# ctu-mrs/mrs_uav_trajectory_generation

Hardware: NVIDIA B200
Metric: optimized+sampled trajectories/sec (10-seg, N=10, fp64) (higher is better)
Workload: dtype f64

## Files before the change

### mrs_uav_trajectory_generation_b200/csrc/cuda_backend.cu

```cuda
#include <cuda_runtime.h>

#include <cub/device/device_scan.cuh>
#include <cub/device/device_select.cuh>
#include <cub/iterator/counting_input_iterator.cuh>
#include <chrono>
#include <cstdlib>
#include <cstring>
#include <map>
#include <mutex>
#include <utility>
#include <vector>
#include <stdexcept>
#include <string>
#include <typeinfo>

#define TG_VERSION_STRING "tg_b200 0.1.0 (sm_100a, fp64, -fmad=false)"

#ifndef TG_JT_REFILL_REP
#define TG_JT_REFILL_REP 2
#endif
#include "tg_kernels.cuh"

namespace {

// ... 2 lines not shown
    cudaError_t e__ = (expr);                                                                            \
    if (e__ != cudaSuccess)                                                                              \
      throw std::runtime_error(std::string(#expr) + ": " + cudaGetErrorString(e__));                     \
  } while (0)

template <class F, class = void>
struct MinBlocksOf {
  static constexpr int value = 1;
};
template <class F>
struct MinBlocksOf<F, decltype((void)F::kMinBlocks)> {
  static constexpr int value = F::kMinBlocks;
};
template <class F>
__global__ void __launch_bounds__(128, MinBlocksOf<F>::value) k_for_each(const F f, const size_t n) {
  const size_t i = (size_t)blockIdx.x * blockDim.x + threadIdx.x;
  if (i < n) f(i);
}

template <class F>
__global__ void __launch_bounds__(128) k_for_each_warp(const F f, const size_t n) {
  const size_t w = (size_t)blockIdx.x * 4 + (threadIdx.x >> 5);
  if (w < n) f(w, (int)(threadIdx.x & 31));
}

static_assert(TG_WARR_DEVICE_STRIDE == 32, "strided scratch kernels run one warp per block");
template <class F>
__global__ void __launch_bounds__(TG_WARR_DEVICE_STRIDE) k_for_each_scratch(const F f, const size_t n) {
  extern __shared__ double smem[];
  const size_t i = (size_t)blockIdx.x * blockDim.x + threadIdx.x;
  if (i < n) f(i, smem + threadIdx.x, (int)blockDim.x);
}

constexpr int kSolveWarps = 4;
template <class D>
__global__ void __launch_bounds__(kSolveWarps * 32) k_solve(const D desc, const size_t inst_begin, const size_t n_inst, const int ws_doubles, double* __restrict__ gws,
                                                            const int skip_oct_ws, const bool skip_thread) {
  extern __shared__ double smem[];
  const int warp = threadIdx.x >> 5, lane = threadIdx.x & 31;
  const size_t gw = (size_t)blockIdx.x * kSolveWarps + warp, nw = (size_t)gridDim.x * kSolveWarps;
  double* ws = gws ? gws + gw * (size_t)ws_doubles : smem + (size_t)warp * ws_doubles;
  for (size_t inst = inst_begin + gw; inst < n_inst; inst += nw) {
    tg::SolveInst I;
    if (!desc.instance(inst, I)) continue;
    if (skip_thread && tg::thread_eligible(I)) continue;
    if (skip_oct_ws > 0 && tg::octet_eligible(I) && tg::octet_ws_doubles(I.S, I.np) <= skip_oct_ws) continue;
// ... 411 lines not shown
    return (double)ms;
  }

  template <class F>
  void for_each(size_t n, const F& f) {
    if (n == 0) return;
    const unsigned block = 128;
    const size_t grid = (n + block - 1) / block;
    prof_begin();
    k_for_each<F><<<(unsigned)grid, block, 0, stream>>>(f, n);
    TG_CUDA_CHECK(cudaGetLastError());
    prof_end(typeid(F).name(), n);
  }
  template <class F>
  void for_each_warp(size_t n, const F& f) {
    if (n == 0) return;
    const size_t grid = (n + 3) / 4;
    prof_begin();
    k_for_each_warp<F><<<(unsigned)grid, 128, 0, stream>>>(f, n);
    TG_CUDA_CHECK(cudaGetLastError());
    prof_end(typeid(F).name(), n);
  }
  template <class F>
  void for_each_scratch(size_t n, const F& f) {
    if (n == 0) return;
    const unsigned block = TG_WARR_DEVICE_STRIDE;
    const size_t grid = (n + block - 1) / block;
    const size_t smem = (size_t)F::kScratch * sizeof(double) * block;
    allow_smem((const void*)k_for_each_scratch<F>, smem);
    prof_begin();
    k_for_each_scratch<F><<<(unsigned)grid, block, smem, stream>>>(f, n);
    TG_CUDA_CHECK(cudaGetLastError());
    prof_end(typeid(F).name(), n);
  }
  void fork(int n) {
    if (profiling) return;
    TG_CUDA_CHECK(cudaEventRecord(ev_fork, stream));
    for (int i = 0; i < n && i < kSideStreams; ++i) TG_CUDA_CHECK(cudaStreamWaitEvent(side[i], ev_fork, 0));
  }
  void join(int n) {
    if (profiling) return;
    for (int i = 0; i < n && i < kSideStreams; ++i) {
      TG_CUDA_CHECK(cudaEventRecord(ev_side[i], side[i]));
      TG_CUDA_CHECK(cudaStreamWaitEvent(stream, ev_side[i], 0));
    }
  }
// ... 293 lines not shown
```

### mrs_uav_trajectory_generation_b200/csrc/tg_kernels.cuh

```cuda
#ifndef TG_KERNELS_CUH_
#define TG_KERNELS_CUH_

#include "tg_common.cuh"
#include "tg_bound.cuh"
#include "tg_plis.cuh"
#include "tg_node.cuh"
#include "tg_poly.cuh"
#include "tg_segment.cuh"
#include "tg_solve.cuh"
#include "tg_solve_octet.cuh"
#include "tg_solve_thread.cuh"

#if defined(__CUDA_ARCH__)
#define TG_ATOMIC_MAX(p, v) atomicMax((p), (v))
#define TG_ATOMIC_ADD(p, v) atomicAdd((p), (v))
#define TG_ATOMIC_ADD_RET(p, v) atomicAdd((p), (v))
#elif defined(__CUDACC__)
#define TG_ATOMIC_MAX(p, v) ((void)0)
#define TG_ATOMIC_ADD(p, v) ((void)0)
#define TG_ATOMIC_ADD_RET(p, v) (0)
#else
static inline void tg_host_atomic_max(int* p, int v) {
  int cur = __atomic_load_n(p, __ATOMIC_RELAXED);
  while (cur < v && !__atomic_compare_exchange_n(p, &cur, v, true, __ATOMIC_RELAXED, __ATOMIC_RELAXED)) {
// ... 25 lines not shown
  double max_dev;
};

struct BatchPtrs {
  int B, totS, totV, r;
  const int* seg_off;
  const int* prob_of_vtx;
  const int* prob_of_seg;
  const double* wp;
  const uint8_t* stop;
  const double* init14;
  uint8_t* vmask;
  double* vval;
  int* vfree;
  int* np;
  int* hbw;
  int* fmax;
  int* stats;
  double *times, *baca, *xeval, *x, *g, *d, *hist_s, *hist_y;
  PlisScalars* opt;
  int* ix;
  int* act_prob[2];
  int* act_vtx[2];
  int* act_seg[2];
  double* recs;
  double* costs;
  double* coef;
  double* maxima;
  ProbState* ps;
  double* xs;
  double* part;
  int xstride, smax;
};

TG_HD int vtx_off(const BatchPtrs& b, int p) { return b.seg_off[p] + p; }

struct PrepareFn {
  BatchPtrs b;
  int from_waypoints;
  TG_HD void operator()(size_t pi) const {
    const int p = (int)pi, s0 = b.seg_off[p], S = b.seg_off[p + 1] - s0, V = S + 1, v0 = s0 + p;
    int hbw = 0, np;
    if (from_waypoints)
      np = build_vertices(V, b.wp + 4 * (size_t)v0, b.stop ? b.stop + v0 : nullptr, b.init14 ? b.init14 + 14 * (size_t)p : nullptr, b.r,
                          b.vmask + v0, b.vval + (size_t)v0 * TG_HALF * TG_D, b.vfree + v0 + p, &hbw);
    else
      np = index_vertices(V, b.vmask + v0, b.vfree + v0 + p, &hbw);
// ... 36 lines not shown
    const int p = b.prob_of_seg[gs];
    const int s0 = b.seg_off[p], S = b.seg_off[p + 1] - s0, i = (int)gs - s0, v0 = s0 + p;
    const double* vpos = b.vval + (size_t)v0 * TG_HALF * TG_D;
    const int stride = TG_HALF * TG_D;
    b.times[gs] = segment_time_euclidean(vpos + (size_t)i * stride, vpos + (size_t)(i + 1) * stride, L);
    b.baca[gs] = segment_time_baca(vpos, stride, i, S + 1, L);
  }
};
struct BacaTotalFn {
  BatchPtrs b;
  TG_HD void operator()(size_t pi) const {
    const int p = (int)pi, s0 = b.seg_off[p], S = b.seg_off[p + 1] - s0;
    double tot = 0.0;
    for (int i = 0; i < S; ++i) tot = tot + b.baca[s0 + i];
    b.ps[p].baca_total = tot;
  }
};

struct SetupBaseFn {
  BatchPtrs b;
  const double* T;
  TG_HD void operator()(size_t gs) const { setup_segment_record(T[gs], b.r, b.recs + gs * TG_REC_SIZE); }
};
template <int STAGE>
struct SetupMellingerFn {
  BatchPtrs b;
  const int* seg_list;
  static constexpr int stage = STAGE;
#ifndef TG_SETUP_ROW_BLOCKS
#define TG_SETUP_ROW_BLOCKS 8
#endif
  static constexpr int kMinBlocks = STAGE ? TG_SETUP_ROW_BLOCKS : 2;
  TG_HD void operator()(size_t item00) const {
    const size_t item0 = stage ? item00 / TG_N : item00;
    const size_t k = item0 / 3;
    const int which = (int)(item0 - k * 3);
    const size_t gs = seg_list ? (size_t)seg_list[k] : k;
    const size_t item = gs * 3 + which;
    const int p = b.prob_of_seg[gs];
    double T = stage ? 0.0 : b.xeval[gs];
    if (b.opt[p].done) return;
    const int S = b.seg_off[p + 1] - b.seg_off[p];
    if (S == 1 && which != 0) return;
    double* rec = b.recs + item * TG_REC_SIZE;
    if (stage) {
      setup_record_hrow(b.r, rec, (int)(item00 - item0 * TG_N));
      return;
    }
    if (which == 1) {
      T = T + 0.1;
      T = dmax(kTimeLowerBound, T);
    } else if (which == 2) {
      const double corr = 0.1 / ((double)S - 1.0);
      T = T - corr;
      T = dmax(kTimeLowerBound, T);
    }
    setup_record_head(T, b.r, rec);
  }
};

struct SolveProblemDesc {
  BatchPtrs b;
  int mellinger;
  double* dp_out;
  const int* dp_off;
  TG_HD bool instance(size_t inst, SolveInst& I) const {
    int p, n;
    if (mellinger == 1) {
      p = b.prob_of_vtx[inst];
      n = (int)inst - vtx_off(b, p);
      if (b.opt[p].done) return false;
    } else {
      p = (int)inst;
      n = 0;
    }
    const int s0 = b.seg_off[p], S = b.seg_off[p + 1] - s0, v0 = s0 + p;
    if (mellinger && S == 1 && n > 0) return false;
    I.S = S;
    I.np = b.np[p];
    I.hbw = b.hbw[p];
// ... 174 lines not shown
    SolveInst I;
    if (!desc.instance(inst, I)) return;
    if (it >= I.S * TG_D) return;
    run_instance(I, inst * (size_t)per_inst + it, it);
  }
  TG_HD void run_instance(const SolveInst& I, size_t item, int it) const {
    const int s = it >> 2, d = it & 3;
    const double* rec = solve_rec(I, s);
    double nd[TG_N], c[TG_N];
#pragma unroll
    for (int k = 0; k < TG_N; ++k) {
      const int v = s + (k >= TG_HALF ? 1 : 0), sl = k - (k >= TG_HALF ? TG_HALF : 0);
      const uint32_t m = I.vmask[v];
      nd[k] = ((m >> sl) & 1u) ? I.vval[((size_t)v * TG_HALF + sl) * TG_D + d] : I.x_out[(size_t)(I.vfree[v] + free_rank(m, sl)) * 4 + d];
    }
    coef_from_endpoints(rec, nd, c);
    if (I.coef_out) {
#pragma unroll
      for (int a = 0; a < TG_N; a += 2) store2(I.coef_out + it * TG_N + a, c[a], c[a + 1]);
    }
    if (I.cost_out) part[item] = cost_partial_rec(I.r, c, rec);
  }
};
struct CoefCostGradFn {
#ifndef TG_COEF_MIN_BLOCKS
#define TG_COEF_MIN_BLOCKS 5
#endif
  static constexpr int kMinBlocks = TG_COEF_MIN_BLOCKS;
  CoefCostFn<SolveProblemDesc> f;
  int p0;
  const int* prob_list;
  TG_HD void operator()(size_t item0) const {
    const BatchPtrs& b = f.desc.b;
    const int p = prob_list ? prob_list[item0 >> 7] : p0 + (int)(item0 >> 7), t = (int)(item0 & 127);
    if (b.opt[p].done) return;
    const int s0 = b.seg_off[p], S = b.seg_off[p + 1] - s0, v0 = s0 + p;
    const int per = S * TG_D, total = (S == 1) ? per : (S + 1) * per;
    SolveInst I;
    I.S = S;
    I.np = 0;
    I.hbw = 0;
    I.fmax = 0;
    I.rec_stride = 3;
    I.r = b.r;
    I.vmask = b.vmask + v0;
    I.vfree = b.vfree + v0 + p;
    I.vval = b.vval + (size_t)v0 * TG_HALF * TG_D;
    I.recs = b.recs + (size_t)s0 * 3 * TG_REC_SIZE;
    I.dp_out = nullptr;
    for (int k = t; k < total; k += 128) {
      const int n = k / per, it = k - n * per;
      I.variant = n;
      I.coef_out = (n == 0) ? b.coef + (size_t)s0 * TG_D * TG_N : nullptr;
      I.cost_out = b.costs + v0 + n;
      I.x_out = b.xs + (size_t)(v0 + n) * (size_t)b.xstride;
      f.run_instance(I, (size_t)(v0 + n) * (size_t)f.per_inst + it, it);
    }
  }
};
template <class D>
struct CostSumFn {
  D desc;
  int per_inst;
  const double* part;
  const int* inst_list = nullptr;
  TG_HD void operator()(size_t k) const {
    const size_t inst = inst_list ? (size_t)inst_list[k] : k;
    SolveInst I;
    if (!desc.instance(inst, I)) return;
    if (!I.cost_out) return;
    const double* pp = part + inst * (size_t)per_inst;
    double total = 0.0;
    for (int it = 0; it < I.S * TG_D; ++it) total += pp[it];
    *I.cost_out = 0.5 * total;
  }
};

TG_HD PlisVectors plis_vectors(const BatchPtrs& b, int p) {
  PlisVectors v;
  const int s0 = b.seg_off[p];
  v.x = b.x + s0;
  v.gf = b.g + s0;
  v.s = b.d + s0;
  v.xeval = b.xeval + s0;
  v.xo = b.hist_s + s0;
  v.go = b.hist_y + s0;
  v.ix = b.ix + s0;
  v.hstride = (size_t)b.totS;
  return v;
}
TG_HD void plis_enlist(const BatchPtrs& b, int p, int buf) {
  const int s0 = b.seg_off[p], S = b.seg_off[p + 1] - s0, v0 = s0 + p;
  int* cnt = b.stats + 9 + 3 * buf;
  const int jp = TG_ATOMIC_ADD_RET(&cnt[0], 1);
  b.act_prob[buf][jp] = p;
  const int jv = TG_ATOMIC_ADD_RET(&cnt[1], S + 1);
  for (int n = 0; n <= S; ++n) b.act_vtx[buf][jv + n] = v0 + n;
  const int js = TG_ATOMIC_ADD_RET(&cnt[2], S);
  for (int i = 0; i < S; ++i) b.act_seg[buf][js + i] = s0 + i;
}
struct PlisBeginFn {
  BatchPtrs b;
  int max_evals;
  TG_HD void operator()(size_t pi) const {
    const int p = (int)pi, s0 = b.seg_off[p], S = b.seg_off[p + 1] - s0;
    if (plis_begin(S, b.opt[p], plis_vectors(b, p), b.times + s0, max_evals)) plis_enlist(b, p, 0);
  }
};
struct PlisAdvanceFn {
  BatchPtrs b;
  int max_evals;
  double f_rel, x_rel;
  const int* prob_list;
  int next_buf;
  TG_HD void operator()(size_t k) const {
    const int p = prob_list ? prob_list[k] : (int)k, s0 = b.seg_off[p], S = b.seg_off[p + 1] - s0;
    PlisScalars& st = b.opt[p];
    if (st.done) return;
    plis_advance(S, st, plis_vectors(b, p), b.costs + vtx_off(b, p), max_evals, f_rel, x_rel, -1.0);
    if (!st.done) {
      TG_ATOMIC_ADD(&b.stats[7], 1);
      plis_enlist(b, p, next_buf);
    }
  }
};
struct PlisFinishFn {
  BatchPtrs b;
  TG_HD void operator()(size_t pi) const {
    const int p = (int)pi, s0 = b.seg_off[p], S = b.seg_off[p + 1] - s0;
    for (int i = 0; i < S; ++i) b.times[s0 + i] = b.xeval[s0 + i];
    ProbState& ps = b.ps[p];
    const PlisScalars& st = b.opt[p];
    ps.nlopt_code = st.code;
    ps.n_evals = st.n_evals;
    ps.n_grads = st.n_evals;
    ps.final_cost = st.f_last;
    if (st.n_evals == 0) ps.scale_done = 1;
    const int code = ps.nlopt_code;
    if (!((code >= 1 && code != 6) || code == -1)) ps.status = kFindNloptRejected;
  }
};

template <int Q>
struct ExtremaFn {
  BatchPtrs b;
// ... 622 lines not shown
```

### mrs_uav_trajectory_generation_b200/csrc/tg_pipeline.hpp

```cpp
#ifndef TG_PIPELINE_HPP_
#define TG_PIPELINE_HPP_

#include <algorithm>
#include <chrono>
#include <cstdio>
#include <cstdlib>
#include <cmath>
#include <cstring>
#include <functional>
#include <memory>
#include <string>
#include <vector>

#include "tg_kernels.cuh"
#include "tg_dfo.cuh"
#include "tg_dfo_generic.cuh"
#include "tg_generic.cuh"

namespace tg {

template <class BE>
class Arena {
 public:
  explicit Arena(BE& be, size_t chunk = (size_t)256 << 20) : be_(be), chunk_(chunk) {}
  ~Arena() {
    for (auto& c : chunks_) be_.dev_free(c.ptr);
  }
  void* alloc_bytes(size_t bytes) {
    bytes = (bytes + 255) & ~(size_t)255;
    if (bytes == 0) bytes = 256;
    while (cur_ < chunks_.size()) {
      Chunk& c = chunks_[cur_];
      if (c.used + bytes <= c.size) {
        void* p = (char*)c.ptr + c.used;
// ... 117 lines not shown
    be_.for_each(totS, tf); launches(1);
    be_.for_each(B, BacaTotalFn{b}); launches(1);
    int stats[16];
    be_.d2h(stats, b.stats, sizeof(stats));
    const int ws = stats[0], ows = stats[2];
    alloc_solution_buffers(b, (size_t)(P.run_time_alloc ? totV : B), stats);
    std::vector<int>& h_np = g.h_np;
    std::vector<int>& h_hbw = g.h_hbw;
    h_np.resize(B);
    h_hbw.resize(B);
    be_.d2h(h_np.data(), b.np, sizeof(int) * B);
    be_.d2h(h_hbw.data(), b.hbw, sizeof(int) * B);
    const std::vector<SolveBucket> buckets = make_buckets(B, g.seg_off.data(), h_np.data(), h_hbw.data(), ws, ows, stats[3]);
    trace_report(" find: prepare + buckets", -1, tf0);
    tf0 = trace_mark();
    if (P.run_time_alloc) {
      time_alloc_core(b, P, stats, &buckets);
      trace_report(" find: time allocation", -1, tf0);
      tf0 = trace_mark();
    } else {
      b.recs = scratch_.template alloc<double>((size_t)totS * TG_REC_SIZE);
    }
    be_.for_each(totS, SetupBaseFn{b, b.times});
    solve_with_outputs((size_t)B, stats, SolveProblemDesc{b, 0, nullptr, nullptr}, b, &buckets, false);
    launches(2);
    int* cap = scratch_.template alloc<int>((size_t)B + 1);
    g.d_smp_off = persist_.template alloc<int>((size_t)B + 1);
    be_.for_each(B, SampleCapFn{b, P.dt, cap}); launches(1);
    be_.exclusive_scan(cap, g.d_smp_off, B); launches(1);
    g.smp_off.resize(B + 1);
    be_.d2h(g.smp_off.data(), g.d_smp_off, sizeof(int) * (B + 1));
    g.totSlots = g.smp_off[B];
    const size_t slots = (size_t)std::max(g.totSlots, 1);
    int* seg_idx = scratch_.template alloc<int>(slots);
    int* smp_prob = scratch_.template alloc<int>(slots);
    double* t_in = scratch_.template alloc<double>(slots);
    g.d_xyzh = persist_.template alloc<double>(slots * 4);
    be_.for_each(B, SampleWalkFn{b, P.dt, g.d_smp_off, seg_idx, t_in});
    be_.for_each(B, SlotProblemFn{B, g.d_smp_off, smp_prob});
    be_.for_each((size_t)g.totSlots, SampleEvalFn{b, g.d_smp_off, smp_prob, seg_idx, t_in, g.d_xyzh, nullptr});
    be_.for_each(B, LengthCheckFn{b, P.dt, P.max_len_factor, P.min_len_factor});
    launches(4);
    if (P.override_heading_atan2) {
      be_.for_each(B, HeadingAtan2Fn{g.d_smp_off, g.d_ps, g.d_xyzh});
      launches(1);
    }
    if (validate) {
// ... 4 lines not shown
    be_.d2h_pinned(g.ps.data(), g.d_ps, sizeof(ProbState) * B);
    trace_report(" find: solve .. state read", -1, tf0);
    if (P.run_time_alloc) {
      int executed = 0;
      be_.d2h(&executed, b.stats + 5, sizeof(int));
      counters.root_finds_executed += executed;
    }
  }
  void account_group(const Group& g, const Params& P) {
    const int B = g.B;
    const std::vector<int>& h_np = g.h_np;
    const std::vector<int>& h_hbw = g.h_hbw;
    for (int p = 0; p < B; ++p) {
      const int S = g.seg_off[p + 1] - g.seg_off[p];
      const int ev = g.ps[p].n_evals;
      const int ng = g.ps[p].n_grads;
      const long long nsolve = (long long)ev + (S == 1 ? 0 : (long long)ng * S) + 1;
      const long long nsetup = (long long)ev * S + (S == 1 ? 0 : (long long)ng * 2 * S) + S;
      const double np_ = h_np[p], bw = h_hbw[p];
      const double f_solve = np_ * (bw * bw + 3.0 * bw) + 4.0 * (2.0 * np_ * 15.0 + 4.0 * np_ * bw);
      const double f_coef = 4.0 * (S * 200.0 + S * 220.0);
      const double nq = TG_N - P.derivative_to_optimize;
      const double f_setup = 3.0 * nq * nq + 525.0 + 4.0 * TG_N * TG_N * TG_N;
      counters.flops_solve += f_solve * (double)nsolve;
      counters.flops_coef += f_coef * (double)nsolve;
      counters.flops_setup += f_setup * (double)nsetup;
      counters.flops_sample += 340.0 * g.ps[p].n_samples;
      counters.mellinger_solves += nsolve - 1;
      counters.evals += ev;
      counters.solves += nsolve;
      counters.segment_setups += nsetup;
      counters.root_finds += (long long)(P.run_time_alloc ? (g.ps[p].n_scale_passes + 1) * 9 * S : 0);
      counters.samples += g.ps[p].n_samples;
    }
  }

  Group* make_group_from_host(const std::vector<int>& members, const int* wp_off, const double* wp, const uint8_t* stop,
                              const double* init14, bool on_device_inputs) {
    groups_.emplace_back(new Group());
    Group& g = *groups_.back();
    const int B = (int)members.size();
    g.B = B;
    g.orig = members;
    g.seg_off.resize(B + 1);
    g.seg_off[0] = 0;
    for (int i = 0; i < B; ++i) g.seg_off[i + 1] = g.seg_off[i] + (wp_off[members[i] + 1] - wp_off[members[i]] - 1);
    g.totS = g.seg_off[B];
    g.totV = g.totS + B;
    alloc_group_outputs(g, init14 != nullptr);
// ... 392 lines not shown
      const int cls = be_.solve_class(ws, ows) * 4096 + (S + 3) / 4;
      if (out.empty() || cls != cls_prev) {
        if (out.size() >= 32) {
          out.assign(1, SolveBucket{0, B, 0, (size_t)seg_off[B] + B, ws_all, ows_all, np_all, 0, 0});
          mixed_single_ = true;
          return out;
        }
        out.push_back(SolveBucket{p, p, (size_t)seg_off[p] + p, 0, 0, 0, 0, 0, cls / 4096});
        cls_prev = cls;
      }
      SolveBucket& k = out.back();
      k.p1 = p + 1;
      k.v1 = (size_t)seg_off[p + 1] + p + 1;
      k.ws = std::max(k.ws, ws);
      k.ows = std::max(k.ows, ows);
      k.np_cap = std::max(k.np_cap, np[p]);
      k.s_cap = std::max(k.s_cap, S);
    }
    mixed_single_ = false;
    return out;
  }
  mutable bool mixed_single_ = false;
  template <class D>
  void solve_with_outputs(size_t n_inst, const int* stats, const D& desc, const BatchPtrs& b, const std::vector<SolveBucket>* buckets = nullptr,
                          bool per_vertex = false) {
    const bool use_thr = thread_solve_for(n_inst);
    const bool thread_all = use_thr && stats[8] == 0;
    if (use_thr) {
      be_.solve_thread(0, n_inst, kThrB * (std::max(b.smax, 1) + 1), desc);
      launches(1);
    }
    be_.skip_thread_eligible = use_thr;
    if (thread_all) {
    } else if (buckets && !buckets->empty()) {
      const bool mixed = mixed_single_;
      size_t a = 0;
      int n_launch = 0;
      while (a < buckets->size()) {
        SolveBucket m = (*buckets)[a];
        size_t e = a + 1;
        while (e < buckets->size() && (*buckets)[e].kernel_cls == m.kernel_cls) {
          const SolveBucket& k = (*buckets)[e];
          m.p1 = k.p1;
          m.v1 = k.v1;
          m.ws = std::max(m.ws, k.ws);
          m.ows = std::max(m.ows, k.ows);
          m.np_cap = std::max(m.np_cap, k.np_cap);
          ++e;
        }
        if (per_vertex) be_.solve(m.v0, m.v1, m.ws, m.ows, m.np_cap, mixed, desc);
        else be_.solve((size_t)m.p0, (size_t)m.p1, m.ws, m.ows, m.np_cap, mixed, desc);
        ++n_launch;
        a = e;
      }
      launches(n_launch - 1);
    } else {
      be_.solve(0, n_inst, stats[0], stats[2], stats[3], stats[6] > 0, desc);
    }
    const int per = 4 * b.smax;
    if (coef_cost_by_problem(n_inst, desc, b, buckets, per)) {
    } else if (buckets && buckets->size() > 1) {
      for (const SolveBucket& k : *buckets) {
        const size_t i0 = per_vertex ? k.v0 : (size_t)k.p0, i1 = per_vertex ? k.v1 : (size_t)k.p1;
        const int items = 4 * std::max(k.s_cap, 1);
        be_.for_each((i1 - i0) * (size_t)items, CoefCostFn<D>{desc, per, b.part, i0, items});
      }
      launches((int)buckets->size() - 1);
    } else {
      be_.for_each(n_inst * (size_t)per, CoefCostFn<D>{desc, per, b.part, 0, per});
    }
    be_.for_each(n_inst, CostSumFn<D>{desc, per, b.part, nullptr});
    launches(2);
  }

  template <class D>
  bool coef_cost_by_problem(size_t, const D&, const BatchPtrs&, const std::vector<SolveBucket>*, int) { return false; }
  bool coef_cost_by_problem(size_t, const SolveProblemDesc& desc, const BatchPtrs& b, const std::vector<SolveBucket>*, int per) {
    if (desc.mellinger != 1) return false;
    be_.for_each((size_t)b.B * 128, CoefCostGradFn{CoefCostFn<SolveProblemDesc>{desc, per, b.part, 0, per}, 0, nullptr});
    return true;
  }

  void time_alloc_core(BatchPtrs& b, const Params& P, const int* stats, const std::vector<SolveBucket>* buckets = nullptr) {
    const int B = b.B, totS = b.totS, totV = b.totV;
    const int mf = (P.max_evals > 0) ? std::min(std::max(P.max_evals, 1), kPlisMfMax) : kPlisMfMax;
    b.xeval = scratch_.template alloc<double>(totS);
    b.x = scratch_.template alloc<double>(totS);
    b.g = scratch_.template alloc<double>(totS);
    b.d = scratch_.template alloc<double>(totS);
    b.ix = scratch_.template alloc<int>(totS);
    b.hist_s = scratch_.template alloc<double>((size_t)mf * totS);
    b.hist_y = scratch_.template alloc<double>((size_t)mf * totS);
    b.opt = scratch_.template alloc<PlisScalars>(B);
    b.recs = scratch_.template alloc<double>((size_t)totS * 3 * TG_REC_SIZE);
    b.costs = scratch_.template alloc<double>(totV);
    b.maxima = scratch_.template alloc<double>((size_t)totS * 9);
    for (int k = 0; k < 2; ++k) {
      b.act_prob[k] = scratch_.template alloc<int>(B);
      b.act_vtx[k] = scratch_.template alloc<int>(totV);
      b.act_seg[k] = scratch_.template alloc<int>(totS);
    }
    be_.dev_memset(b.stats + 9, 0, 6 * sizeof(int));
    be_.for_each(B, PlisBeginFn{b, P.max_evals}); launches(1);
    const int eval_cap = (P.max_evals > 0 ? P.max_evals : 1000) + 64;
    int cnt[3] = {B, totV, totS};
    const bool lists_ok = thread_solve_for((size_t)totV) && stats[8] == 0;
    for (int e = 0; e < eval_cap; ++e) {
      const int buf = e & 1, nbuf = buf ^ 1;
      const bool sparse = lists_ok && e > 0 && (size_t)cnt[0] * 2 < (size_t)B;
      be_.dev_memset(b.stats + 7, 0, sizeof(int));
      be_.dev_memset(b.stats + 9 + 3 * nbuf, 0, 3 * sizeof(int));
      if (sparse) {
        const SolveProblemDesc desc{b, 1, nullptr, nullptr};
        const int per = 4 * b.smax;
        be_.for_each((size_t)cnt[2] * 3, SetupMellingerFn<0>{b, b.act_seg[buf]});
        be_.for_each((size_t)cnt[2] * 3 * TG_N, SetupMellingerFn<1>{b, b.act_seg[buf]});
        if ((size_t)cnt[1] >= list_octet_below) {
          be_.solve_thread(0, (size_t)cnt[1], kThrB * (std::max(b.smax, 1) + 1), SolveProblemListDesc{desc, b.act_vtx[buf]});
        } else {
          be_.skip_thread_eligible = false;
          be_.solve(0, (size_t)cnt[1], stats[0], stats[2], stats[3], stats[6] > 0, SolveProblemListDesc{desc, b.act_vtx[buf]});
        }
        be_.for_each((size_t)cnt[0] * 128, CoefCostGradFn{CoefCostFn<SolveProblemDesc>{desc, per, b.part, 0, per}, 0, b.act_prob[buf]});
        be_.for_each((size_t)cnt[1], CostSumFn<SolveProblemDesc>{desc, per, b.part, b.act_vtx[buf]});
        be_.for_each((size_t)cnt[0], PlisAdvanceFn{b, P.max_evals, P.f_rel, P.x_rel, b.act_prob[buf], nbuf});
        launches(6);
      } else {
        be_.for_each((size_t)totS * 3, SetupMellingerFn<0>{b, nullptr});
        be_.for_each((size_t)totS * 3 * TG_N, SetupMellingerFn<1>{b, nullptr});
        solve_with_outputs((size_t)totV, stats, SolveProblemDesc{b, 1, nullptr, nullptr}, b, buckets, true);
        be_.for_each(B, PlisAdvanceFn{b, P.max_evals, P.f_rel, P.x_rel, nullptr, nbuf});
        launches(4);
      }
      counters.mellinger_launches += 1;
      run_deferred();
      int back[8];
      be_.d2h(back, b.stats + 7, sizeof(back));
      if (back[0] == 0) break;
      cnt[0] = back[2 + 3 * nbuf];
      cnt[1] = back[3 + 3 * nbuf];
      cnt[2] = back[4 + 3 * nbuf];
    }
    be_.for_each(B, PlisFinishFn{b}); launches(1);
    scale_loop(b, P.limits);
  }

  bool time_alloc_batch(int B, const int* vtx_off, const uint8_t* vmask, const double* vval, double* times, const Params& P, double* coef,
                        int* nlopt_code, int* n_evals, int* n_scale_passes, double* final_cost) {
    scratch_.reset();
    std::vector<int> so(B + 1);
    for (int p = 0; p <= B; ++p) so[p] = vtx_off[p] - p;
    for (int p = 0; p < B; ++p)
      if (so[p + 1] - so[p] < 1) return false;
    Bare bb = bare_batch(B, so.data(), P.derivative_to_optimize);
    BatchPtrs& b = bb.b;
    b.vmask = scratch_.template alloc<uint8_t>(b.totV);
    b.vval = scratch_.template alloc<double>((size_t)b.totV * TG_HALF * TG_D);
    b.vfree = scratch_.template alloc<int>((size_t)b.totV + B);
    b.np = scratch_.template alloc<int>(B);
    b.hbw = scratch_.template alloc<int>(B);
    b.fmax = scratch_.template alloc<int>(B);
    b.times = scratch_.template alloc<double>(b.totS);
    b.coef = scratch_.template alloc<double>((size_t)b.totS * TG_D * TG_N);
    be_.h2d(b.vmask, vmask, b.totV);
// ... 887 lines not shown
    double* d_ws = scratch_.template alloc<double>((size_t)std::max<long long>(ws_tot, 1));
    double* d_cost = scratch_.template alloc<double>(B);
    b.vmask = scratch_.template alloc<uint8_t>(totV);
    b.vval = scratch_.template alloc<double>((size_t)totV * H * TG_D);
    b.vfree = scratch_.template alloc<int>(gv.vfree.size());
    b.np = scratch_.template alloc<int>(B);
    b.hbw = scratch_.template alloc<int>(B);
    b.times = scratch_.template alloc<double>(totS);
    b.coef = scratch_.template alloc<double>((size_t)totS * TG_D * N);
    b.recs = scratch_.template alloc<double>((size_t)totS * 3 * gen::Rec<N>::kSize);
    b.costs = scratch_.template alloc<double>(totV);
    b.maxima = scratch_.template alloc<double>((size_t)totS * 9);
    b.xeval = scratch_.template alloc<double>(totS);
    b.x = scratch_.template alloc<double>(totS);
    b.g = scratch_.template alloc<double>(totS);
    b.d = scratch_.template alloc<double>(totS);
    b.ix = scratch_.template alloc<int>(totS);
    b.hist_s = scratch_.template alloc<double>((size_t)mf * totS);
    b.hist_y = scratch_.template alloc<double>((size_t)mf * totS);
    b.opt = scratch_.template alloc<PlisScalars>(B);
    for (int k = 0; k < 2; ++k) {
      b.act_prob[k] = scratch_.template alloc<int>(B);
      b.act_vtx[k] = scratch_.template alloc<int>(totV);
      b.act_seg[k] = scratch_.template alloc<int>(totS);
    }
    be_.h2d(d_vtx_off, vtx_off, sizeof(int) * ((size_t)B + 1));
    be_.h2d(d_ws_inst, ws_inst.data(), sizeof(long long) * totV);
    be_.h2d(d_ws_prob, ws_prob.data(), sizeof(long long) * B);
    be_.h2d(b.vmask, vmask, totV);
    be_.h2d(b.vval, vval, sizeof(double) * (size_t)totV * H * TG_D);
    be_.h2d(b.vfree, gv.vfree.data(), sizeof(int) * gv.vfree.size());
    be_.h2d(b.np, gv.np.data(), sizeof(int) * B);
    be_.h2d(b.hbw, gv.hbw.data(), sizeof(int) * B);
    be_.h2d(b.times, times, sizeof(double) * totS);
    be_.dev_memset(b.stats + 9, 0, 6 * sizeof(int));
    be_.for_each(B, PlisBeginFn{b, P.max_evals}); launches(1);
    const int eval_cap = (P.max_evals > 0 ? P.max_evals : 1000) + 64;
    for (int e = 0; e < eval_cap; ++e) {
      const int nbuf = (e & 1) ^ 1;
      be_.dev_memset(b.stats + 7, 0, sizeof(int));
      be_.dev_memset(b.stats + 9 + 3 * nbuf, 0, 3 * sizeof(int));
      be_.for_each((size_t)totS * 3, gen::MellingerHeadFn<N>{b});
      be_.for_each((size_t)totS * 3 * N, gen::MellingerHrowFn<N>{b});
      be_.for_each_warp((size_t)totV, gen::MellingerSolveFn<N>{b, d_ws_inst, d_ws});
      be_.for_each(B, PlisAdvanceFn{b, P.max_evals, P.f_rel, P.x_rel, nullptr, nbuf});
      launches(4);
      counters.mellinger_launches += 1;
      int running = 0;
      be_.d2h(&running, b.stats + 7, sizeof(int));
      if (running == 0) break;
    }
    be_.for_each(B, PlisFinishFn{b}); launches(1);
    scale_loop_n<N>(b, P.limits);
    be_.for_each((size_t)totS, gen::RecordHeadFn<N>{b.r, b.times, b.recs});
    be_.for_each((size_t)totS * N, gen::RecordHrowFn<N>{b.recs});
    be_.for_each_warp((size_t)B, gen::SolveFn<N>{b.r, d_vtx_off, b.vmask, b.vfree, b.vval, b.np, b.hbw, b.recs, d_ws_prob, d_ws, b.coef, d_cost});
    launches(3);
    std::vector<ProbState> ps(B);
    be_.d2h(ps.data(), b.ps, sizeof(ProbState) * B);
    for (int p = 0; p < B; ++p) {
      if (nlopt_code) nlopt_code[p] = ps[p].nlopt_code;
      if (n_evals) n_evals[p] = ps[p].n_evals;
      if (n_scale_passes) n_scale_passes[p] = ps[p].n_scale_passes;
      if (final_cost) final_cost[p] = ps[p].final_cost;
// ... 517 lines not shown
```

### mrs_uav_trajectory_generation_b200/csrc/tg_segment.cuh

```cuda
#ifndef TG_SEGMENT_CUH_
#define TG_SEGMENT_CUH_

#include "tg_common.cuh"

namespace tg {

TG_HD void inverse5(const double (&Din)[5][5], double (&out)[5][5]) {
  double lu[5][5];
  int perm[5];
#pragma unroll
  for (int i = 0; i < 5; ++i) {
    perm[i] = i;
#pragma unroll
    for (int j = 0; j < 5; ++j) lu[i][j] = Din[i][j];
  }
#pragma unroll
  for (int k = 0; k < 5; ++k) {
    int piv = k;
    double best = dabs(lu[k][k]);
#pragma unroll
    for (int i = k + 1; i < 5; ++i) {
      const double a = dabs(lu[i][k]);
      if (a > best) { best = a; piv = i; }
    }
// ... 128 lines not shown
      if (b < 5) {
        bool have = false;
        s = 0.0;
        if (b >= R) { s = W[(b >= R) ? b - R : 0] * a_inv[b]; have = true; }
#pragma unroll
        for (int k = 5; k < TG_N; ++k) {
          const double t = W[k - R] * X[k - 5][b];
          s = have ? s + t : t;
          have = true;
        }
      } else {
        s = W[5 - R] * Dinv[0][b - 5];
#pragma unroll
        for (int k = 6; k < TG_N; ++k) s = s + W[k - R] * Dinv[k - 5][b - 5];
      }
      hrow[b] = s;
    }
#pragma unroll
    for (int b = 0; b < TG_N; b += 2) store2(rec + TG_REC_H + a * TG_N + b, hrow[b], hrow[b + 1]);
  }
}

template <int R>
TG_HD void setup_record_head_r(double T, double* __restrict__ rec) {
  constexpr int NQ = TG_N - R;
  constexpr int EMAX = (TG_N - 1 - R) * 2 + 1;
  double pw[EMAX];
  tgdm::powers(T, EMAX, pw);
  {
    double qt[36];
#pragma unroll
    for (int e = 0; e < 36; ++e) qt[e] = 0.0;
#pragma unroll
    for (int i = 0; i < NQ; ++i)
#pragma unroll
      for (int j = i; j < NQ; ++j) {
        const int e = i + j + 1;
        qt[tg_qtri(i, j)] = bcoef(R, i + R) * bcoef(R, j + R) * pw[e - 1] * 2.0 / (double)e;
      }
#pragma unroll
    for (int e = 0; e < 36; e += 2) store2(rec + TG_REC_Q + e, qt[e], qt[e + 1]);
  }
  double tp[TG_N];
  tp[0] = 1.0;
  tp[1] = T;
#pragma unroll
  for (int m = 2; m < TG_N; ++m) tp[m] = tp[m - 1] * T;
  const bool tzero = dabs(T) < TG_DBL_EPSILON;
  double Dm[5][5], Cm[5][5];
#pragma unroll
  for (int k = 0; k < 5; ++k)
#pragma unroll
    for (int j = 0; j < 5; ++j) {
      Dm[k][j] = tzero ? 0.0 : bcoef(k, 5 + j) * tp[5 + j - k];
      Cm[k][j] = (j < k) ? 0.0 : ((j == k) ? bcoef(k, k) : (tzero ? 0.0 : bcoef(k, j) * tp[j - k]));
    }
  double Dinv[5][5];
  inverse5(Dm, Dinv);
  const double a_inv[5] = {1.0 / 1.0, 1.0 / 1.0, 1.0 / 2.0, 1.0 / 6.0, 1.0 / 24.0};
  double X[5][5];
#pragma unroll
  for (int i = 0; i < 5; ++i)
#pragma unroll
    for (int j = 0; j < 5; ++j) {
      double m = (-Dinv[i][0]) * Cm[0][j];
#pragma unroll
      for (int k = 1; k <= j; ++k) m = m + (-Dinv[i][k]) * Cm[k][j];
      X[i][j] = m * a_inv[j];
    }
#pragma unroll
  for (int e = 0; e < 50; e += 2) {
    const double v0 = (e < 25) ? Dinv[e / 5][e % 5] : X[(e - 25) / 5][(e - 25) % 5];
    const double v1 = (e + 1 < 25) ? Dinv[(e + 1) / 5][(e + 1) % 5] : X[(e + 1 - 25) / 5][(e + 1 - 25) % 5];
    store2(rec + e, v0, v1);
  }
}
template <int R>
TG_HD void setup_record_hrow_r(double* __restrict__ rec, int a) {
  constexpr int NQ = TG_N - R;
  const double a_inv[5] = {1.0 / 1.0, 1.0 / 1.0, 1.0 / 2.0, 1.0 / 6.0, 1.0 / 24.0};
  const double* __restrict__ Dinv = rec + TG_REC_DINV;
  const double* __restrict__ X = rec + TG_REC_X;
  const double* __restrict__ Qt = rec + TG_REC_Q;
  double col[5];
#pragma unroll
  for (int k = 0; k < 5; ++k) col[k] = (a < 5) ? X[k * 5 + a] : Dinv[k * 5 + (a - 5)];
  const double ainv_a = (a < 5) ? a_inv[a < 5 ? a : 0] : 0.0;
  double W[NQ];
#pragma unroll
  for (int b = 0; b < NQ; ++b) {
    bool have = false;
    double s = 0.0;
    if (a < 5 && a >= R) {
      s = ainv_a * Qt[tg_qsym(a - R, b)];
      have = true;
    }
#pragma unroll
    for (int k = 5; k < TG_N; ++k) {
// ... 12 lines not shown
      s = 0.0;
      if (b >= R) { s = W[(b >= R) ? b - R : 0] * a_inv[b]; have = true; }
#pragma unroll
      for (int k = 5; k < TG_N; ++k) {
        const double t = W[k - R] * X[(k - 5) * 5 + b];
        s = have ? s + t : t;
        have = true;
      }
    } else {
      s = W[5 - R] * Dinv[0 * 5 + (b - 5)];
#pragma unroll
      for (int k = 6; k < TG_N; ++k) s = s + W[k - R] * Dinv[(k - 5) * 5 + (b - 5)];
    }
    hrow[b] = s;
  }
#pragma unroll
  for (int b = 0; b < TG_N; b += 2) store2(rec + TG_REC_H + a * TG_N + b, hrow[b], hrow[b + 1]);
}
TG_HD void setup_record_head(double T, int r, double* __restrict__ rec) {
  if (r == 2) setup_record_head_r<2>(T, rec);
  else if (r == 3) setup_record_head_r<3>(T, rec);
  else setup_record_head_r<4>(T, rec);
}
TG_HD void setup_record_hrow(int r, double* __restrict__ rec, int a) {
  if (r == 2) setup_record_hrow_r<2>(rec, a);
  else if (r == 3) setup_record_hrow_r<3>(rec, a);
  else setup_record_hrow_r<4>(rec, a);
}

TG_HD_NOINLINE void setup_segment_record(double T, int r, double* __restrict__ rec) {
  if (r == 2) setup_segment_record_r<2>(T, rec);
  else if (r == 3) setup_segment_record_r<3>(T, rec);
  else setup_segment_record_r<4>(T, rec);
}

}

#endif
```

Before: 403,300.

## Fuse Mellinger eval epilogue into one block-per-problem kernel with next-iteration setup

Replaces the per-iteration chain of coef/cost, cost-sum, PLIS advance and record-setup launches with a single block-per-problem kernel. Each block computes coefficients and costs, reduces partial costs in shared memory, advances the optimizer, and, if the problem continues, builds the next iteration's segment records in shared memory and writes them out. Initial records are set up once before the loop. This cuts launches and global round-trips per iteration, at the cost of heavy shared-memory use per block and block-level synchronisation.

```diff
diff --git a/mrs_uav_trajectory_generation_b200/csrc/cuda_backend.cu b/mrs_uav_trajectory_generation_b200/csrc/cuda_backend.cu
--- a/mrs_uav_trajectory_generation_b200/csrc/cuda_backend.cu
+++ b/mrs_uav_trajectory_generation_b200/csrc/cuda_backend.cu
@@ -48,6 +48,12 @@
 __global__ void __launch_bounds__(128) k_for_each_warp(const F f, const size_t n) {
   const size_t w = (size_t)blockIdx.x * 4 + (threadIdx.x >> 5);
   if (w < n) f(w, (int)(threadIdx.x & 31));
+}
+
+template <class F>
+__global__ void __launch_bounds__(F::kThreads, MinBlocksOf<F>::value) k_for_each_block(const F f) {
+  __shared__ typename F::Shared sm;
+  f(blockIdx.x, (int)threadIdx.x, sm);
 }
 
 static_assert(TG_WARR_DEVICE_STRIDE == 32, "strided scratch kernels run one warp per block");
@@ -505,6 +511,14 @@
     prof_end(typeid(F).name(), n);
   }
   template <class F>
+  void for_each_block(size_t n, const F& f) {
+    if (n == 0) return;
+    prof_begin();
+    k_for_each_block<F><<<(unsigned)n, F::kThreads, 0, stream>>>(f);
+    TG_CUDA_CHECK(cudaGetLastError());
+    prof_end(typeid(F).name(), n);
+  }
+  template <class F>
   void for_each_scratch(size_t n, const F& f) {
     if (n == 0) return;
     const unsigned block = TG_WARR_DEVICE_STRIDE;
diff --git a/mrs_uav_trajectory_generation_b200/csrc/tg_kernels.cuh b/mrs_uav_trajectory_generation_b200/csrc/tg_kernels.cuh
--- a/mrs_uav_trajectory_generation_b200/csrc/tg_kernels.cuh
+++ b/mrs_uav_trajectory_generation_b200/csrc/tg_kernels.cuh
@@ -71,7 +71,6 @@
   int* ix;
   int* act_prob[2];
   int* act_vtx[2];
-  int* act_seg[2];
   double* recs;
   double* costs;
   double* coef;
@@ -154,21 +153,29 @@
   const double* T;
   TG_HD void operator()(size_t gs) const { setup_segment_record(T[gs], b.r, b.recs + gs * TG_REC_SIZE); }
 };
+TG_HD double mellinger_record_time(double T, int which, int S) {
+  if (which == 1) {
+    T = T + 0.1;
+    T = dmax(kTimeLowerBound, T);
+  } else if (which == 2) {
+    const double corr = 0.1 / ((double)S - 1.0);
+    T = T - corr;
+    T = dmax(kTimeLowerBound, T);
+  }
+  return T;
+}
 template <int STAGE>
 struct SetupMellingerFn {
   BatchPtrs b;
-  const int* seg_list;
   static constexpr int stage = STAGE;
 #ifndef TG_SETUP_ROW_BLOCKS
 #define TG_SETUP_ROW_BLOCKS 8
 #endif
   static constexpr int kMinBlocks = STAGE ? TG_SETUP_ROW_BLOCKS : 2;
   TG_HD void operator()(size_t item00) const {
-    const size_t item0 = stage ? item00 / TG_N : item00;
-    const size_t k = item0 / 3;
-    const int which = (int)(item0 - k * 3);
-    const size_t gs = seg_list ? (size_t)seg_list[k] : k;
-    const size_t item = gs * 3 + which;
+    const size_t item = stage ? item00 / TG_N : item00;
+    const size_t gs = item / 3;
+    const int which = (int)(item - gs * 3);
     const int p = b.prob_of_seg[gs];
     double T = stage ? 0.0 : b.xeval[gs];
     if (b.opt[p].done) return;
@@ -176,18 +183,10 @@
     if (S == 1 && which != 0) return;
     double* rec = b.recs + item * TG_REC_SIZE;
     if (stage) {
-      setup_record_hrow(b.r, rec, (int)(item00 - item0 * TG_N));
+      setup_record_hrow(b.r, rec, (int)(item00 - item * TG_N));
       return;
     }
-    if (which == 1) {
-      T = T + 0.1;
-      T = dmax(kTimeLowerBound, T);
-    } else if (which == 2) {
-      const double corr = 0.1 / ((double)S - 1.0);
-      T = T - corr;
-      T = dmax(kTimeLowerBound, T);
-    }
-    setup_record_head(T, b.r, rec);
+    setup_record_head(mellinger_record_time(T, which, S), b.r, rec);
   }
 };
 
@@ -408,42 +407,6 @@
     if (I.cost_out) part[item] = cost_partial_rec(I.r, c, rec);
   }
 };
-struct CoefCostGradFn {
-#ifndef TG_COEF_MIN_BLOCKS
-#define TG_COEF_MIN_BLOCKS 5
-#endif
-  static constexpr int kMinBlocks = TG_COEF_MIN_BLOCKS;
-  CoefCostFn<SolveProblemDesc> f;
-  int p0;
-  const int* prob_list;
-  TG_HD void operator()(size_t item0) const {
-    const BatchPtrs& b = f.desc.b;
-    const int p = prob_list ? prob_list[item0 >> 7] : p0 + (int)(item0 >> 7), t = (int)(item0 & 127);
-    if (b.opt[p].done) return;
-    const int s0 = b.seg_off[p], S = b.seg_off[p + 1] - s0, v0 = s0 + p;
-    const int per = S * TG_D, total = (S == 1) ? per : (S + 1) * per;
-    SolveInst I;
-    I.S = S;
-    I.np = 0;
-    I.hbw = 0;
-    I.fmax = 0;
-    I.rec_stride = 3;
-    I.r = b.r;
-    I.vmask = b.vmask + v0;
-    I.vfree = b.vfree + v0 + p;
-    I.vval = b.vval + (size_t)v0 * TG_HALF * TG_D;
-    I.recs = b.recs + (size_t)s0 * 3 * TG_REC_SIZE;
-    I.dp_out = nullptr;
-    for (int k = t; k < total; k += 128) {
-      const int n = k / per, it = k - n * per;
-      I.variant = n;
-      I.coef_out = (n == 0) ? b.coef + (size_t)s0 * TG_D * TG_N : nullptr;
-      I.cost_out = b.costs + v0 + n;
-      I.x_out = b.xs + (size_t)(v0 + n) * (size_t)b.xstride;
-      f.run_instance(I, (size_t)(v0 + n) * (size_t)f.per_inst + it, it);
-    }
-  }
-};
 template <class D>
 struct CostSumFn {
   D desc;
@@ -477,13 +440,11 @@
 }
 TG_HD void plis_enlist(const BatchPtrs& b, int p, int buf) {
   const int s0 = b.seg_off[p], S = b.seg_off[p + 1] - s0, v0 = s0 + p;
-  int* cnt = b.stats + 9 + 3 * buf;
+  int* cnt = b.stats + 9 + 2 * buf;
   const int jp = TG_ATOMIC_ADD_RET(&cnt[0], 1);
   b.act_prob[buf][jp] = p;
   const int jv = TG_ATOMIC_ADD_RET(&cnt[1], S + 1);
   for (int n = 0; n <= S; ++n) b.act_vtx[buf][jv + n] = v0 + n;
-  const int js = TG_ATOMIC_ADD_RET(&cnt[2], S);
-  for (int i = 0; i < S; ++i) b.act_seg[buf][js + i] = s0 + i;
 }
 struct PlisBeginFn {
   BatchPtrs b;
@@ -493,20 +454,117 @@
     if (plis_begin(S, b.opt[p], plis_vectors(b, p), b.times + s0, max_evals)) plis_enlist(b, p, 0);
   }
 };
+TG_HD bool plis_step(const BatchPtrs& b, int p, int max_evals, double f_rel, double x_rel, int next_buf) {
+  const int s0 = b.seg_off[p], S = b.seg_off[p + 1] - s0;
+  PlisScalars& st = b.opt[p];
+  if (st.done) return false;
+  plis_advance(S, st, plis_vectors(b, p), b.costs + vtx_off(b, p), max_evals, f_rel, x_rel, -1.0);
+  if (st.done) return false;
+  TG_ATOMIC_ADD(&b.stats[7], 1);
+  plis_enlist(b, p, next_buf);
+  return true;
+}
 struct PlisAdvanceFn {
   BatchPtrs b;
   int max_evals;
   double f_rel, x_rel;
   const int* prob_list;
   int next_buf;
-  TG_HD void operator()(size_t k) const {
-    const int p = prob_list ? prob_list[k] : (int)k, s0 = b.seg_off[p], S = b.seg_off[p + 1] - s0;
-    PlisScalars& st = b.opt[p];
-    if (st.done) return;
-    plis_advance(S, st, plis_vectors(b, p), b.costs + vtx_off(b, p), max_evals, f_rel, x_rel, -1.0);
-    if (!st.done) {
-      TG_ATOMIC_ADD(&b.stats[7], 1);
-      plis_enlist(b, p, next_buf);
+  TG_HD void operator()(size_t k) const { plis_step(b, prob_list ? prob_list[k] : (int)k, max_evals, f_rel, x_rel, next_buf); }
+};
+
+#ifndef TG_EPI_THREADS
+#define TG_EPI_THREADS 128
+#endif
+constexpr int kEpiThreads = TG_EPI_THREADS;
+constexpr int kEpiPartCap = 1024;
+constexpr int kEpiSegs = 10;
+#if defined(__CUDA_ARCH__)
+#define TG_BLOCK_PHASE(t) for (int tg_once_ = 0; tg_once_ < 1; ++tg_once_, __syncthreads())
+#else
+#define TG_BLOCK_PHASE(t) for (int t = 0; t < kEpiThreads; ++t)
+#endif
+struct alignas(16) EvalEpilogueShared {
+  union {
+    double part[kEpiPartCap];
+    double rec[3 * kEpiSegs * TG_REC_SIZE];
+  };
+  double total[kEpiThreads];
+  int runs;
+};
+struct EvalEpilogueFn {
+  typedef EvalEpilogueShared Shared;
+  static constexpr int kThreads = kEpiThreads;
+  static constexpr int kMinBlocks = 512 / kEpiThreads;
+  BatchPtrs b;
+  int max_evals;
+  double f_rel, x_rel;
+  const int* prob_list;
+  int next_buf;
+  TG_HD void operator()(size_t blk, int t, Shared& sm) const {
+    const int p = prob_list ? prob_list[blk] : (int)blk;
+    if (b.opt[p].done) return;
+    const int s0 = b.seg_off[p], S = b.seg_off[p + 1] - s0, v0 = s0 + p;
+    const int per = S * TG_D, nvar = (S == 1) ? 1 : S + 1;
+    SolveInst I;
+    I.S = S;
+    I.np = 0;
+    I.hbw = 0;
+    I.fmax = 0;
+    I.rec_stride = 3;
+    I.r = b.r;
+    I.vmask = b.vmask + v0;
+    I.vfree = b.vfree + v0 + p;
+    I.vval = b.vval + (size_t)v0 * TG_HALF * TG_D;
+    I.recs = b.recs + (size_t)s0 * 3 * TG_REC_SIZE;
+    I.dp_out = nullptr;
+    const CoefCostFn<SolveProblemDesc> cf{SolveProblemDesc{b, 1, nullptr, nullptr}, 0, sm.part, 0, 0};
+    const int vpp = imax(1, imin(kEpiThreads, kEpiPartCap / per)), ipp = imin(per, kEpiPartCap);
+    for (int n0 = 0; n0 < nvar; n0 += vpp) {
+      const int nv = imin(vpp, nvar - n0);
+      for (int i0 = 0; i0 < per; i0 += ipp) {
+        const int ni = imin(ipp, per - i0);
+        TG_BLOCK_PHASE(t) {
+          for (int k = t; k < nv * ni; k += kEpiThreads) {
+            const int dn = k / ni, it = i0 + (k - dn * ni), n = n0 + dn;
+            I.variant = n;
+            I.coef_out = (n == 0) ? b.coef + (size_t)s0 * TG_D * TG_N : nullptr;
+            I.cost_out = b.costs + v0 + n;
+            I.x_out = b.xs + (size_t)(v0 + n) * (size_t)b.xstride;
+            cf.run_instance(I, (size_t)k, it);
+          }
+        }
+        TG_BLOCK_PHASE(t) {
+          if (t < nv) {
+            double total = (i0 == 0) ? 0.0 : sm.total[t];
+            for (int k = 0; k < ni; ++k) total += sm.part[t * ni + k];
+            sm.total[t] = total;
+            if (i0 + ni == per) b.costs[v0 + n0 + t] = 0.5 * total;
+          }
+        }
+      }
+    }
+    TG_BLOCK_PHASE(t) {
+      if (t == 0) sm.runs = plis_step(b, p, max_evals, f_rel, x_rel, next_buf) ? 1 : 0;
+    }
+    if (!sm.runs) return;
+    double* recs = b.recs + (size_t)s0 * 3 * TG_REC_SIZE;
+    for (int c0 = 0; c0 < S; c0 += kEpiSegs) {
+      const int nrec = (S == 1) ? 1 : 3 * imin(kEpiSegs, S - c0);
+      TG_BLOCK_PHASE(t) {
+        for (int h = t; h < 2 * nrec; h += kEpiThreads) {
+          const int q = h >> 1, k = q / 3, which = q - 3 * k;
+          setup_record_head_part(mellinger_record_time(b.xeval[s0 + c0 + k], which, S), b.r, sm.rec + q * TG_REC_SIZE, h & 1);
+        }
+      }
+      TG_BLOCK_PHASE(t) {
+        for (int k = t; k < nrec * TG_N; k += kEpiThreads) setup_record_hrow(b.r, sm.rec + (k / TG_N) * TG_REC_SIZE, k % TG_N);
+      }
+      TG_BLOCK_PHASE(t) {
+        const Dbl2* src = reinterpret_cast<const Dbl2*>(sm.rec);
+        Dbl2* dst = reinterpret_cast<Dbl2*>(recs + (size_t)c0 * 3 * TG_REC_SIZE);
+        for (int k = t; k < nrec * (TG_REC_SIZE / 2); k += kEpiThreads) dst[k] = src[k];
+      }
     }
   }
 };
diff --git a/mrs_uav_trajectory_generation_b200/csrc/tg_pipeline.hpp b/mrs_uav_trajectory_generation_b200/csrc/tg_pipeline.hpp
--- a/mrs_uav_trajectory_generation_b200/csrc/tg_pipeline.hpp
+++ b/mrs_uav_trajectory_generation_b200/csrc/tg_pipeline.hpp
@@ -8,8 +8,10 @@
 #include <cmath>
 #include <cstring>
 #include <functional>
+#include <limits>
 #include <memory>
 #include <string>
+#include <type_traits>
 #include <vector>
 
 #include "tg_kernels.cuh"
@@ -173,7 +175,7 @@
       b.recs = scratch_.template alloc<double>((size_t)totS * TG_REC_SIZE);
     }
     be_.for_each(totS, SetupBaseFn{b, b.times});
-    solve_with_outputs((size_t)B, stats, SolveProblemDesc{b, 0, nullptr, nullptr}, b, &buckets, false);
+    solve_with_outputs((size_t)B, stats, SolveProblemDesc{b, 0, nullptr, nullptr}, b, &buckets);
     launches(2);
     int* cap = scratch_.template alloc<int>((size_t)B + 1);
     g.d_smp_off = persist_.template alloc<int>((size_t)B + 1);
@@ -224,9 +226,10 @@
       const double f_coef = 4.0 * (S * 200.0 + S * 220.0);
       const double nq = TG_N - P.derivative_to_optimize;
       const double f_setup = 3.0 * nq * nq + 525.0 + 4.0 * TG_N * TG_N * TG_N;
+      const long long nsetup_launched = (ev > 0 ? (S == 1 ? 1 : 3 * S) : 0) + S;
       counters.flops_solve += f_solve * (double)nsolve;
-      counters.flops_coef += f_coef * (double)nsolve;
-      counters.flops_setup += f_setup * (double)nsetup;
+      counters.flops_coef += f_coef;
+      counters.flops_setup += f_setup * (double)nsetup_launched;
       counters.flops_sample += 340.0 * g.ps[p].n_samples;
       counters.mellinger_solves += nsolve - 1;
       counters.evals += ev;
@@ -665,8 +668,7 @@
   }
   mutable bool mixed_single_ = false;
   template <class D>
-  void solve_with_outputs(size_t n_inst, const int* stats, const D& desc, const BatchPtrs& b, const std::vector<SolveBucket>* buckets = nullptr,
-                          bool per_vertex = false) {
+  void solve_instances(size_t n_inst, const int* stats, const D& desc, const BatchPtrs& b, const std::vector<SolveBucket>* buckets, bool per_vertex) {
     const bool use_thr = thread_solve_for(n_inst);
     const bool thread_all = use_thr && stats[8] == 0;
     if (use_thr) {
@@ -700,13 +702,15 @@
     } else {
       be_.solve(0, n_inst, stats[0], stats[2], stats[3], stats[6] > 0, desc);
     }
+  }
+  template <class D>
+  void solve_with_outputs(size_t n_inst, const int* stats, const D& desc, const BatchPtrs& b, const std::vector<SolveBucket>* buckets = nullptr) {
+    solve_instances(n_inst, stats, desc, b, buckets, false);
     const int per = 4 * b.smax;
-    if (coef_cost_by_problem(n_inst, desc, b, buckets, per)) {
-    } else if (buckets && buckets->size() > 1) {
+    if (buckets && buckets->size() > 1) {
       for (const SolveBucket& k : *buckets) {
-        const size_t i0 = per_vertex ? k.v0 : (size_t)k.p0, i1 = per_vertex ? k.v1 : (size_t)k.p1;
         const int items = 4 * std::max(k.s_cap, 1);
-        be_.for_each((i1 - i0) * (size_t)items, CoefCostFn<D>{desc, per, b.part, i0, items});
+        be_.for_each((size_t)(k.p1 - k.p0) * (size_t)items, CoefCostFn<D>{desc, per, b.part, (size_t)k.p0, items});
       }
       launches((int)buckets->size() - 1);
     } else {
@@ -716,12 +720,24 @@
     launches(2);
   }
 
-  template <class D>
-  bool coef_cost_by_problem(size_t, const D&, const BatchPtrs&, const std::vector<SolveBucket>*, int) { return false; }
-  bool coef_cost_by_problem(size_t, const SolveProblemDesc& desc, const BatchPtrs& b, const std::vector<SolveBucket>*, int per) {
-    if (desc.mellinger != 1) return false;
-    be_.for_each((size_t)b.B * 128, CoefCostGradFn{CoefCostFn<SolveProblemDesc>{desc, per, b.part, 0, per}, 0, nullptr});
-    return true;
+  template <class B2, class = void>
+  struct HasBlockLaunch : std::false_type {};
+  template <class B2>
+  struct HasBlockLaunch<B2, decltype((void)&B2::template for_each_block<EvalEpilogueFn>)> : std::true_type {};
+  template <class F>
+  struct HostBlockFn {
+    F f;
+    void operator()(size_t i) const {
+      std::unique_ptr<typename F::Shared> sm(new typename F::Shared);
+      double* d = reinterpret_cast<double*>(sm.get());
+      for (size_t k = 0; k < sizeof(typename F::Shared) / sizeof(double); ++k) d[k] = std::numeric_limits<double>::quiet_NaN();
+      f(i, 0, *sm);
+    }
+  };
+  template <class F>
+  void for_each_block(size_t n, const F& f) {
+    if constexpr (HasBlockLaunch<BE>::value) be_.for_each_block(n, f);
+    else be_.for_each(n, HostBlockFn<F>{f});
   }
 
   void time_alloc_core(BatchPtrs& b, const Params& P, const int* stats, const std::vector<SolveBucket>* buckets = nullptr) {
@@ -741,48 +757,41 @@
     for (int k = 0; k < 2; ++k) {
       b.act_prob[k] = scratch_.template alloc<int>(B);
       b.act_vtx[k] = scratch_.template alloc<int>(totV);
-      b.act_seg[k] = scratch_.template alloc<int>(totS);
-    }
-    be_.dev_memset(b.stats + 9, 0, 6 * sizeof(int));
+    }
+    be_.dev_memset(b.stats + 9, 0, 4 * sizeof(int));
     be_.for_each(B, PlisBeginFn{b, P.max_evals}); launches(1);
     const int eval_cap = (P.max_evals > 0 ? P.max_evals : 1000) + 64;
-    int cnt[3] = {B, totV, totS};
+    int cnt[2] = {B, totV};
     const bool lists_ok = thread_solve_for((size_t)totV) && stats[8] == 0;
+    const SolveProblemDesc desc{b, 1, nullptr, nullptr};
+    be_.for_each((size_t)totS * 3, SetupMellingerFn<0>{b});
+    be_.for_each((size_t)totS * 3 * TG_N, SetupMellingerFn<1>{b});
+    launches(2);
     for (int e = 0; e < eval_cap; ++e) {
       const int buf = e & 1, nbuf = buf ^ 1;
       const bool sparse = lists_ok && e > 0 && (size_t)cnt[0] * 2 < (size_t)B;
       be_.dev_memset(b.stats + 7, 0, sizeof(int));
-      be_.dev_memset(b.stats + 9 + 3 * nbuf, 0, 3 * sizeof(int));
+      be_.dev_memset(b.stats + 9 + 2 * nbuf, 0, 2 * sizeof(int));
       if (sparse) {
-        const SolveProblemDesc desc{b, 1, nullptr, nullptr};
-        const int per = 4 * b.smax;
-        be_.for_each((size_t)cnt[2] * 3, SetupMellingerFn<0>{b, b.act_seg[buf]});
-        be_.for_each((size_t)cnt[2] * 3 * TG_N, SetupMellingerFn<1>{b, b.act_seg[buf]});
         if ((size_t)cnt[1] >= list_octet_below) {
           be_.solve_thread(0, (size_t)cnt[1], kThrB * (std::max(b.smax, 1) + 1), SolveProblemListDesc{desc, b.act_vtx[buf]});
         } else {
           be_.skip_thread_eligible = false;
           be_.solve(0, (size_t)cnt[1], stats[0], stats[2], stats[3], stats[6] > 0, SolveProblemListDesc{desc, b.act_vtx[buf]});
         }
-        be_.for_each((size_t)cnt[0] * 128, CoefCostGradFn{CoefCostFn<SolveProblemDesc>{desc, per, b.part, 0, per}, 0, b.act_prob[buf]});
-        be_.for_each((size_t)cnt[1], CostSumFn<SolveProblemDesc>{desc, per, b.part, b.act_vtx[buf]});
-        be_.for_each((size_t)cnt[0], PlisAdvanceFn{b, P.max_evals, P.f_rel, P.x_rel, b.act_prob[buf], nbuf});
-        launches(6);
+        for_each_block((size_t)cnt[0], EvalEpilogueFn{b, P.max_evals, P.f_rel, P.x_rel, b.act_prob[buf], nbuf});
       } else {
-        be_.for_each((size_t)totS * 3, SetupMellingerFn<0>{b, nullptr});
-        be_.for_each((size_t)totS * 3 * TG_N, SetupMellingerFn<1>{b, nullptr});
-        solve_with_outputs((size_t)totV, stats, SolveProblemDesc{b, 1, nullptr, nullptr}, b, buckets, true);
-        be_.for_each(B, PlisAdvanceFn{b, P.max_evals, P.f_rel, P.x_rel, nullptr, nbuf});
-        launches(4);
+        solve_instances((size_t)totV, stats, desc, b, buckets, true);
+        for_each_block((size_t)B, EvalEpilogueFn{b, P.max_evals, P.f_rel, P.x_rel, nullptr, nbuf});
       }
+      launches(2);
       counters.mellinger_launches += 1;
       run_deferred();
-      int back[8];
+      int back[6];
       be_.d2h(back, b.stats + 7, sizeof(back));
       if (back[0] == 0) break;
-      cnt[0] = back[2 + 3 * nbuf];
-      cnt[1] = back[3 + 3 * nbuf];
-      cnt[2] = back[4 + 3 * nbuf];
+      cnt[0] = back[2 + 2 * nbuf];
+      cnt[1] = back[3 + 2 * nbuf];
     }
     be_.for_each(B, PlisFinishFn{b}); launches(1);
     scale_loop(b, P.limits);
@@ -1716,7 +1725,6 @@
     for (int k = 0; k < 2; ++k) {
       b.act_prob[k] = scratch_.template alloc<int>(B);
       b.act_vtx[k] = scratch_.template alloc<int>(totV);
-      b.act_seg[k] = scratch_.template alloc<int>(totS);
     }
     be_.h2d(d_vtx_off, vtx_off, sizeof(int) * ((size_t)B + 1));
     be_.h2d(d_ws_inst, ws_inst.data(), sizeof(long long) * totV);
@@ -1727,13 +1735,13 @@
     be_.h2d(b.np, gv.np.data(), sizeof(int) * B);
     be_.h2d(b.hbw, gv.hbw.data(), sizeof(int) * B);
     be_.h2d(b.times, times, sizeof(double) * totS);
-    be_.dev_memset(b.stats + 9, 0, 6 * sizeof(int));
+    be_.dev_memset(b.stats + 9, 0, 4 * sizeof(int));
     be_.for_each(B, PlisBeginFn{b, P.max_evals}); launches(1);
     const int eval_cap = (P.max_evals > 0 ? P.max_evals : 1000) + 64;
     for (int e = 0; e < eval_cap; ++e) {
       const int nbuf = (e & 1) ^ 1;
       be_.dev_memset(b.stats + 7, 0, sizeof(int));
-      be_.dev_memset(b.stats + 9 + 3 * nbuf, 0, 3 * sizeof(int));
+      be_.dev_memset(b.stats + 9 + 2 * nbuf, 0, 2 * sizeof(int));
       be_.for_each((size_t)totS * 3, gen::MellingerHeadFn<N>{b});
       be_.for_each((size_t)totS * 3 * N, gen::MellingerHrowFn<N>{b});
       be_.for_each_warp((size_t)totV, gen::MellingerSolveFn<N>{b, d_ws_inst, d_ws});
diff --git a/mrs_uav_trajectory_generation_b200/csrc/tg_segment.cuh b/mrs_uav_trajectory_generation_b200/csrc/tg_segment.cuh
--- a/mrs_uav_trajectory_generation_b200/csrc/tg_segment.cuh
+++ b/mrs_uav_trajectory_generation_b200/csrc/tg_segment.cuh
@@ -174,25 +174,25 @@
 }
 
 template <int R>
-TG_HD void setup_record_head_r(double T, double* __restrict__ rec) {
+TG_HD void setup_record_q_r(double T, double* __restrict__ rec) {
   constexpr int NQ = TG_N - R;
   constexpr int EMAX = (TG_N - 1 - R) * 2 + 1;
   double pw[EMAX];
   tgdm::powers(T, EMAX, pw);
-  {
-    double qt[36];
-#pragma unroll
-    for (int e = 0; e < 36; ++e) qt[e] = 0.0;
-#pragma unroll
-    for (int i = 0; i < NQ; ++i)
-#pragma unroll
-      for (int j = i; j < NQ; ++j) {
-        const int e = i + j + 1;
-        qt[tg_qtri(i, j)] = bcoef(R, i + R) * bcoef(R, j + R) * pw[e - 1] * 2.0 / (double)e;
-      }
-#pragma unroll
-    for (int e = 0; e < 36; e += 2) store2(rec + TG_REC_Q + e, qt[e], qt[e + 1]);
-  }
+  double qt[36];
+#pragma unroll
+  for (int e = 0; e < 36; ++e) qt[e] = 0.0;
+#pragma unroll
+  for (int i = 0; i < NQ; ++i)
+#pragma unroll
+    for (int j = i; j < NQ; ++j) {
+      const int e = i + j + 1;
+      qt[tg_qtri(i, j)] = bcoef(R, i + R) * bcoef(R, j + R) * pw[e - 1] * 2.0 / (double)e;
+    }
+#pragma unroll
+  for (int e = 0; e < 36; e += 2) store2(rec + TG_REC_Q + e, qt[e], qt[e + 1]);
+}
+TG_HD void setup_record_dx_r(double T, double* __restrict__ rec) {
   double tp[TG_N];
   tp[0] = 1.0;
   tp[1] = T;
@@ -226,6 +226,11 @@
     const double v1 = (e + 1 < 25) ? Dinv[(e + 1) / 5][(e + 1) % 5] : X[(e + 1 - 25) / 5][(e + 1 - 25) % 5];
     store2(rec + e, v0, v1);
   }
+}
+template <int R>
+TG_HD void setup_record_head_r(double T, double* __restrict__ rec) {
+  setup_record_q_r<R>(T, rec);
+  setup_record_dx_r(T, rec);
 }
 template <int R>
 TG_HD void setup_record_hrow_r(double* __restrict__ rec, int a) {
@@ -284,6 +289,12 @@
   else if (r == 3) setup_record_head_r<3>(T, rec);
   else setup_record_head_r<4>(T, rec);
 }
+TG_HD void setup_record_head_part(double T, int r, double* __restrict__ rec, int part) {
+  if (part == 1) setup_record_dx_r(T, rec);
+  else if (r == 2) setup_record_q_r<2>(T, rec);
+  else if (r == 3) setup_record_q_r<3>(T, rec);
+  else setup_record_q_r<4>(T, rec);
+}
 TG_HD void setup_record_hrow(int r, double* __restrict__ rec, int a) {
   if (r == 2) setup_record_hrow_r<2>(rec, a);
   else if (r == 3) setup_record_hrow_r<3>(rec, a);
```

Result: slower. 384,900, median of 6 (-4.6%).
